# Xharlie/BtcDet

Measured on AMD Instinct MI355X. Metric: scenes/s fwd+bwd KITTI-Car bs=2/GPU (BtcDet hot path), higher is better.
Workload: dtype f32

## Files before the change

btcdet_amd/_lib.py:

```python
import ctypes
import os

import numpy as np
import torch

_HERE = os.path.dirname(os.path.abspath(__file__))
LIB_PATH = os.path.join(_HERE, "libbtcdet_hip.so")
_lib = None

c_i32p = ctypes.POINTER(ctypes.c_int32)
c_f32p = ctypes.POINTER(ctypes.c_float)
vp = ctypes.c_void_p
ci = ctypes.c_int
sz = ctypes.c_size_t

MODE_SUBM, MODE_CONV, MODE_TRANSPOSE = 0, 1, 2


class BtcHipError(RuntimeError):
    pass


class BtcOccConfig(ctypes.Structure):
    _fields_ = [("batch", ctypes.c_int32), ("grid", ctypes.c_int32 * 3), ("sphere_grid", ctypes.c_int32 * 3),
# ... 109 lines not shown
                              sz, vp]),
    "btc_occ_loss_bwd": (ci, [vp, vp, vp, vp, vp, vp, vp, vp, ci, ctypes.c_longlong, ctypes.c_float, vp, vp, vp, vp, vp]),
    "btc_occ_loss_fwd_total": (ci, [vp, vp, vp, vp, vp, vp, vp, vp, ci, ctypes.c_longlong, ctypes.c_float, ctypes.c_float, ctypes.c_float, vp, vp,
                                    vp, sz, vp]),
    "btc_occ_loss_bwd_total": (ci, [vp, vp, vp, vp, vp, vp, vp, vp, ci, ctypes.c_longlong, ctypes.c_float, vp, vp, vp, vp, vp]),
    "btc_dense_split_fwd": (ci, [vp, vp, ci, ci, ci, vp, vp, vp, vp]),
    "btc_occ_prob": (ci, [vp, vp, ci, ctypes.c_longlong, vp, vp]),
    "btc_dense_split_bwd": (ci, [vp, vp, vp, ci, ci, ci, vp, vp, vp]),
    "btc_cat_pad_fwd": (ci, [vp, ci, vp, ci, ctypes.c_longlong, ci, ci, vp, vp]),
    "btc_cat_pad_bwd": (ci, [vp, ci, ctypes.c_longlong, ci, vp, ci, vp, ci, vp]),
    "btc_sumsq2_ws_bytes": (sz, []),
    "btc_sumsq2_fwd": (ci, [vp, ctypes.c_longlong, ci, ctypes.c_double, vp, ctypes.c_longlong, ci, ctypes.c_double, vp, vp, sz, vp]),
    "btc_sumsq2_bwd": (ci, [vp, ctypes.c_longlong, ci, ctypes.c_float, vp, vp, ctypes.c_longlong, ci, ctypes.c_float, vp, vp, vp]),
    "btc_bn_ws_bytes": (sz, [ci]),
    "btc_bn_relu_fwd": (ci, [vp, ci, ci, vp, vp, vp, vp, vp, ctypes.c_float, ctypes.c_float, ci, ci, vp, vp, vp, vp, sz, vp]),
    "btc_spin": (ci, [ci, vp]),
    "btc_bn_relu_bwd": (ci, [vp, vp, vp, ci, ci, vp, vp, vp, ci, ci, vp, vp, vp, vp, sz, vp]),
    "btc_bn_relu_fwd_bf16": (ci, [vp, ci, ci, vp, vp, vp, vp, vp, ctypes.c_float, ctypes.c_float, ci, ci, vp, vp, vp, vp, sz, vp]),
    "btc_bn_relu_bwd_bf16": (ci, [vp, vp, vp, ci, ci, vp, vp, vp, ci, ci, vp, vp, vp, vp, sz, vp]),
    "btc_ball_query": (ci, [vp, vp, vp, vp, ci, ci, ctypes.c_float, ctypes.c_float, ci, vp, vp]),
    "btc_group_points": (ci, [vp, vp, vp, vp, ci, ci, ci, ci, vp, vp]),
    "btc_group_points_grad": (ci, [vp, vp, vp, vp, ci, ci, ci, ci, ci, vp, vp]),
    "btc_furthest_point_sampling": (ci, [vp, ci, ci, ci, vp, vp, vp]),
    "btc_three_nn": (ci, [vp, vp, vp, vp, ci, ci, vp, vp, vp]),
    "btc_three_interpolate": (ci, [vp, vp, vp, ci, ci, vp, vp]),
    "btc_three_interpolate_grad": (ci, [vp, vp, vp, ci, ci, ci, vp, vp]),
    "btc_bn_fuse_ws_bytes": (sz, []),
    "btc_conv_bn_relu_fwd": (ci, [ci, vp, vp, vp, vp, vp, ci, ci, ci, ci, vp, vp, vp, vp, vp, vp, ctypes.c_float, ctypes.c_float, ci, vp, vp, vp, vp, sz, vp, vp]),
    "btc_conv_bn_relu_fwd_src": (ci, [ci, vp, ctypes.c_longlong, vp, vp, vp, vp, ci, ci, ci, ci, vp, vp, vp, vp, vp, vp, ctypes.c_float, ctypes.c_float, ci, vp, vp, vp, vp, sz, vp, vp]),
    "btc_col_sum": (ci, [vp, ci, ci, vp, vp, sz, vp]),
    "btc_col_sum_bf16": (ci, [vp, ci, ci, vp, vp, sz, vp]),
    "btc_occ_targets_ws_bytes": (sz, [ctypes.POINTER(BtcOccConfig)]),
    "btc_occ_backproject_lut": (ci, [ctypes.POINTER(BtcOccConfig), vp, vp]),
    "btc_occ_targets": (ci, [ctypes.POINTER(BtcOccConfig), vp, vp, vp, ci, ci, ci, vp, vp, vp, vp, ci, vp, vp,
                             ctypes.POINTER(BtcOccBuffers), vp, sz, vp]),
}

EXPORTED_SYMBOLS = tuple(_SIGS.keys())

_INFER_SIGS = {
    "btc_conv_bn_eval_fwd": (ci, [ci, vp, ctypes.c_longlong, vp, vp, vp, vp, ci, ci, ci, ci, vp, vp, vp, vp, ctypes.c_float, ci, vp, vp]),
    "btc_det_select_nms_ws_bytes": (sz, [ci, ci]),
    "btc_det_select_nms": (ci, [vp, vp, ci, ci, ci, ci, ci, ctypes.c_float, ctypes.c_float, ci, ci, ci, vp, vp, vp, vp, sz, vp]),
    "btc_det_finish": (ci, [vp, vp, ci, ci, ci, ci, ci, ci, vp, vp, vp, vp, ci, vp, ci, ci, vp, ci, ci, c_f32p, ci, vp, vp, vp, vp, vp, vp]),
    "btc_occ_metrics_ws_bytes": (sz, [ci, ci]),
    "btc_occ_metrics": (ci, [vp, vp, vp, vp, ctypes.c_longlong, vp, vp, vp, ctypes.c_longlong, vp, vp, ci, ci, ci, vp, vp, sz, vp]),
    "btc_kitti_overlaps": (ci, [vp, vp, vp, vp, vp, c_i32p, ci, vp, vp, vp]),
    "btc_kitti_match_tp": (ci, [vp, vp, vp, vp, vp, vp, vp, c_i32p, ci, ci, ci, ci, ci, ci, vp, vp, vp]),
    "btc_kitti_match_stats_ws_bytes": (sz, [ci, ci, ci, ci, ci]),
    "btc_kitti_match_stats": (ci, [vp, vp, vp, vp, vp, vp, vp, vp, vp, vp, vp, c_i32p, ci, ci, ci, ci, ci, ci, ci, vp, vp, vp, sz, vp]),
}

INFER_EXPORTED_SYMBOLS = tuple(_INFER_SIGS.keys())

_AUGMENT_SIGS = {
    "btc_augment_ws_bytes": (sz, [ci, ci, ci]),
    "btc_augment_batch": (ci, [vp, ci, ci, vp, ci, vp, vp, vp, ctypes.c_longlong, vp, vp, vp, vp, ci, ctypes.c_longlong, vp, vp,
                               ctypes.c_longlong, vp, vp, vp, vp, sz, vp]),
    "btc_world_transform": (ci, [vp, ci, ci, vp, ci, vp, vp, vp, vp]),
}

AUGMENT_EXPORTED_SYMBOLS = tuple(_AUGMENT_SIGS.keys())

_BESTMATCH_SIGS = {
    "btc_place_templates": (ci, [vp, ctypes.c_longlong, vp, vp, vp, vp, vp, ci, ci, vp, vp, ctypes.c_longlong, ci, vp, vp]),
}

BESTMATCH_EXPORTED_SYMBOLS = tuple(_BESTMATCH_SIGS.keys())

_FRAMES_SIGS = {
    "btc_fov_crop_ws_bytes": (sz, [ci, ci]),
    "btc_fov_crop": (ci, [vp, ci, ci, vp, ci, vp, ci, vp, vp, vp, vp, sz, vp]),
}

FRAMES_EXPORTED_SYMBOLS = tuple(_FRAMES_SIGS.keys())

_GTDB_SIGS = {
    "btc_cut_objects_ws_bytes": (sz, [ci, ci, ci, ci]),
    "btc_cut_objects": (ci, [vp, ci, ci, vp, ci, vp, vp, vp, ci, ci, ci, vp, vp, vp, vp, sz, vp]),
}

GTDB_EXPORTED_SYMBOLS = tuple(_GTDB_SIGS.keys())


def lib():
    global _lib
    if _lib is None:
        if not os.path.exists(LIB_PATH):
            raise BtcHipError(
                f"{LIB_PATH} not found: build it with `python -c 'import __graft_entry__ as g; g.build()'` "
                f"or `make -C btcdet_amd/csrc` (there is no CPU fallback for the hot path)")
        L = ctypes.CDLL(LIB_PATH)
        for name, (res, args) in (list(_SIGS.items()) + list(_INFER_SIGS.items()) + list(_AUGMENT_SIGS.items()) + list(_BESTMATCH_SIGS.items()) +
                                  list(_FRAMES_SIGS.items()) + list(_GTDB_SIGS.items())):
            fn = getattr(L, name)
            fn.restype = res
            fn.argtypes = args
        for kv in filter(None, os.environ.get("BTC_TUNE", "").split(",")):
            k, v = kv.split("=")
            if L.btc_tune_set(int(k), int(v)) != 0:
                raise BtcHipError("BTC_TUNE: bad entry %r" % kv)
        _lib = L
    return _lib


_fast = False


def fast():
    global _fast
    if _fast is False:
        _fast = None
        if os.environ.get("BTC_FASTPATH", "1") != "0":
            try:
                lib()
                from . import _btcfast
                if _btcfast.abi_version() == lib().btc_version():
                    _fast = _btcfast
            except ImportError:
                _fast = None
    return _fast


def check(rc, what):
    if rc != 0:
        msg = lib().btc_last_error().decode("utf-8", "replace")
        raise BtcHipError(f"{what} failed (code {rc}): {msg}")


_raw_stream = torch._C._cuda_getCurrentRawStream
_cur_device = torch._C._cuda_getDevice


def stream_ptr():
    return _raw_stream(_cur_device())


def ptr(t):
    if t is None:
        return None
    if not (t.is_cuda and t.is_contiguous()):
        raise BtcHipError("expected a contiguous tensor on the GPU (HIP) device")
    return t.data_ptr()


_I3_CACHE = {}


def i3(v):
    if isinstance(v, (int, np.integer)):
        key = (int(v),) * 3
    else:
        key = tuple(int(x) for x in np.asarray(v).reshape(-1))
        if len(key) != 3:
            raise BtcHipError(f"expected 3 values, got {v!r}")
    a = _I3_CACHE.get(key)
    if a is None:
        a = np.ascontiguousarray(np.array(key, dtype=np.int32))
        a.setflags(write=False)
        a_ptr = a.ctypes.data_as(c_i32p)
        _I3_CACHE[key] = a
        _I3P_CACHE[id(a)] = (a, a_ptr)
    return a


_I3P_CACHE = {}


def i3p(a):
    hit = _I3P_CACHE.get(id(a))
    if hit is not None and hit[0] is a:
        return hit[1]
    return a.ctypes.data_as(c_i32p)


def f32p(a):
    return a.ctypes.data_as(c_f32p)
# ... 5 lines not shown
```

btcdet_amd/backbones_3d.py:

```python
import os
from functools import partial

import torch
import torch.nn as nn

from . import spconv


def post_act_block(in_channels, out_channels, kernel_size, indice_key=None, stride=1, padding=0, conv_type='subm',
                   norm_fn=None, defaultvalue=1.0, activation=nn.ReLU):
    if conv_type == 'subm':
        conv = spconv.SubMConv3d(in_channels, out_channels, kernel_size, bias=False, indice_key=indice_key)
    elif conv_type == 'subm2d':
        conv = spconv.SubMConv2d(in_channels, out_channels, kernel_size, bias=False, indice_key=indice_key)
    elif conv_type == 'spconv':
        conv = spconv.SparseConv3d(in_channels, out_channels, kernel_size, stride=stride, padding=padding, bias=False,
                                   indice_key=indice_key)
    elif conv_type == 'fixspconv':
        conv = fixSparseConv3d(in_channels, out_channels, kernel_size, stride=stride, padding=padding, bias=False,
                               indice_key=indice_key, defaultvalue=defaultvalue)
        conv.requires_grad_(False)
    elif conv_type == 'spdeconv':
        conv = spconv.SparseConvTranspose3d(in_channels, out_channels, kernel_size, stride=stride, padding=padding,
                                            bias=False, indice_key=indice_key)
# ... 226 lines not shown

    def _stage(self, stage, x, ready):
        sl = ready[0].stage_slices.get(id(stage)) if ready is not None else None
        if sl is not None:
            chain = stage._chain_plan(x, ready[1][sl[0]:sl[1]])
            if chain is not None:
                return stage._run_chain(x, *chain)
        return stage(x)

    def _stages(self, stages, x, ready):
        for stage in stages:
            x = self._stage(stage, x, ready)
        return x

    def _build_occ_net(self, kind, i):
        n = self.occ_code_num
        key = 'spconv%d' % (i + 1)
        pad = 1 if i < 3 else (1, 1, 1)
        kw = {'maxpool': dict(k=3, conv_type='maxpool'), 'weight': dict(k=3, conv_type='spconv'),
              'fix': dict(k=3, conv_type='fixspconv', defaultvalue=1.0 / 27),
              'avgpool': dict(k=2, conv_type='fixspconv', defaultvalue=1)}[kind]
        k = kw.pop('k')
        setattr(self, 'occ_conv%d' % (i + 1), spconv.SparseSequential(
            post_act_block(n, n, k, norm_fn=None, stride=2, padding=pad, indice_key=key, **kw)))

    def _build_combine_net(self, norm_fn, c, comb_type):
        sp = dict(stride=2, conv_type='spconv')
        self.down2 = _seq([(c[1], c[1], 3, dict(padding=1, indice_key='spconv3', **sp)),
                           (c[1], c[2], 3, dict(padding=(0, 1, 1), indice_key='spconv4', **sp))], norm_fn)
        self.down3 = _seq([(c[2], c[2], 3, dict(padding=(0, 1, 1), indice_key='spconv4', **sp))], norm_fn)
        cat = c[2] * 2 + c[3]
        if comb_type == "big_combine":
            self.down_combine = _seq([(cat, c[3] * 2, 3, dict(padding=1, indice_key='subm4')),
                                      (c[3] * 2, c[3] * 2, 3, dict(padding=1, indice_key='subm4'))], norm_fn)
        elif comb_type == "combine":
            self.down_combine = _seq([(cat, c[3] * 2, 3, dict(padding=1, indice_key='subm4')),
                                      (c[3] * 2, c[3] * 2, 3, dict(stride=[1, 2, 2], padding=(1, 1, 1), indice_key='spconv5',
                                                                   conv_type='spconv')),
                                      (c[3] * 2, c[3] * 2, 3, dict(padding=1, indice_key='subm5'))], norm_fn)
        elif comb_type == "big_bev_combine":
            self.squeezeBev = _seq([(c[4], c[3], (2, 1, 1), dict(stride=(2, 1, 1), padding=0, indice_key='subm_down2',
                                                                  conv_type='spconv'))], norm_fn)
            self.down_combine = _seq([(cat + c[3], c[3] * 2, 3, dict(padding=1, indice_key='subm4')),
                                      (c[3] * 2, c[3] * 2, 3, dict(padding=1, indice_key='subm4'))], norm_fn)

    @staticmethod
    def sparse_cat(input_lst, pad=False):
        xrep, xocc = input_lst
        if pad:
            from .spconv import ops as sp_ops
            xrep.features = sp_ops.cat_features(xrep.features, xocc.features)
        else:
            xrep.features = torch.cat((xrep.features, xocc.features.to(xrep.features.dtype)), dim=1)
        return xrep

    @staticmethod
    def apply_att(x, att_conv):
        a = att_conv(x)
        x.features = x.features * a.features + x.features
        return x

    def suqeeze(self, feat, i, kind):
        if kind == "None":
            return None
        if kind == "3D":
            return feat
        conv = getattr(self, "squeeze_z_conv{}".format(i), None)
        dense = feat.dense()
        B, C, Z, Y, X = list(dense.shape)
        inds = torch.unique(torch.cat([feat.indices[..., 0:1], feat.indices[..., 2:]], dim=-1), dim=0).long()
        pix = dense.reshape(B, C * Z, Y, X)[inds[..., 0], :, inds[..., 1], inds[..., 2]]
        return conv(spconv.SparseConvTensor(features=pix, indices=inds.int(), spatial_shape=[Y, X], batch_size=B)).dense()

    @staticmethod
    def compress_height(t):
        d = t.dense()
        N, C, D, H, W = d.shape
        return d.view(N, C * D, H, W)

    def res_combine(self, x2, x3, x4, bev, out_feat_type="combine", ready=None):
        if getattr(self, "down3", None) is None:
            return None
        x2, x3 = self._stage(self.down2, x2, ready), self._stage(self.down3, x3, ready)
        if out_feat_type == "big_bev_combine":
            bev2d = self.compress_height(self._stage(self.squeezeBev, bev, ready))
            x4.features = torch.cat((x2.features, x3.features, x4.features,
                                     _BevGather.apply(bev2d, x4.indices, tuple(x4.spatial_shape), x4.batch_size).to(x4.features.dtype)), dim=1)
        else:
            x4.features = torch.cat((x2.features, x3.features, x4.features), dim=1)
        return self._stage(self.down_combine, x4, ready)

    @staticmethod
    def _coords_i32(batch_dict):
        from .vfe import i32_twin
        coords = batch_dict['voxel_coords']
        tw = i32_twin(batch_dict, coords)
        return tw if tw is not None else coords.int()

    def prefetch_geometry(self, batch_dict):
        coords = self._coords_i32(batch_dict)
        if not coords.is_cuda or coords.shape[0] == 0:
            return batch_dict
        indice_dict = {}
        walk = self._walk_geometry(coords, batch_dict['batch_size'], indice_dict, allow_async=False)
        if isinstance(walk, tuple) and walk[0] == "done":
            batch_dict['det_geometry'] = (coords, indice_dict, walk)
        return batch_dict

    def forward(self, batch_dict):
        coords = self._coords_i32(batch_dict)
        feats = batch_dict['voxel_features']
        if self.feature_dtype is not None and feats.shape[1] % 16 == 0:
            feats = feats.to(self.feature_dtype)
        bs = batch_dict['batch_size']
        x = spconv.SparseConvTensor(features=feats, indices=coords, spatial_shape=self.sparse_shape, batch_size=bs)
        pre = batch_dict.pop('det_geometry', None)
        if pre is not None and pre[0] is coords:
            x.indice_dict = pre[1]
            walk = pre[2]
        else:
            walk = self._walk_geometry(coords, bs, x.indice_dict)
        n_occ = len(self.occ_conv_exec)
        ready = None
        if FAST_STAGES and isinstance(walk, tuple) and walk[0] == "done":
            ready = self._finish_walk(walk, x.indice_dict)
        merge_first = ready is not None and not (n_occ > 0 and self.occ_conv_exec[0])
        x1 = _to_feature_dtype(self._stage(self.conv1, x, ready), self.feature_dtype)
        if merge_first:
            x1 = self._stage(self.conv1_combine, x1, ready)
        occ = None
        if n_occ > 0:
            occ = spconv.SparseConvTensor(features=batch_dict["occ_voxel_features"], indices=coords,
                                          spatial_shape=self.sparse_shape, batch_size=bs)
            occ.indice_dict["__geometry_cache__"] = x.indice_dict.setdefault("__geometry_cache__", {})
            if self.occ_conv_exec[0]:
                x1 = self.sparse_cat([x1, occ], pad=not self.out_att[0])
                if self.out_att[0]:
                    x1 = self.apply_att(x1, self.att_conv1)
        if not merge_first:
            x1 = self._stage(self.conv1_combine, x1, ready)
        if ready is None:
            ready = self._finish_walk(walk, x.indice_dict)
            if not FAST_STAGES:
                ready = None
        levels = [x1]
        cur = x1
        for lvl in (1, 2, 3):
            if not (n_occ > lvl):
                cur = self._stages([getattr(self, 'conv%d' % (lvl + 1)), getattr(self, 'conv%d_combine' % (lvl + 1))], cur, ready)
                levels.append(cur)
                continue
            cur = self._stage(getattr(self, 'conv%d' % (lvl + 1)), cur, ready)
            if n_occ > lvl:
                occ = getattr(self, 'occ_conv%d' % (lvl + 1))(occ)
                if self.occ_conv_exec[lvl]:
                    cur = self.sparse_cat([cur, occ], pad=not self.out_att[lvl])
                    if self.out_att[lvl]:
                        cur = self.apply_att(cur, getattr(self, 'att_conv%d' % (lvl + 1)))
            cur = self._stage(getattr(self, 'conv%d_combine' % (lvl + 1)), cur, ready)
            levels.append(cur)
        x1, x2, x3, x4 = levels
        out = self._stage(self.conv_out, x4, ready)
        batch_dict.update({'encoded_spconv_tensor': out, 'encoded_spconv_tensor_stride': 8})
        batch_dict['__level_rows__'] = {'det_L0': int(x1.features.shape[0]), 'det_L1': int(x2.features.shape[0]),
                                        'det_L2': int(x3.features.shape[0]), 'det_L3': int(x4.features.shape[0]),
                                        'det_out': int(out.features.shape[0])}
        batch_dict.update({'multi_scale_3d_features': {
            'x_conv1': self.suqeeze(x1, 1, self.out_feat_type[0]),
            'x_conv2': self.suqeeze(x2, 2, self.out_feat_type[1]),
            'x_conv3': self.suqeeze(x3, 3, self.out_feat_type[2]),
            'x_conv4': self.suqeeze(x4, 4, self.out_feat_type[3]),
            'x_combine': self.res_combine(x2, x3, x4, out, out_feat_type=self.out_feat_type[4], ready=ready),
# ... 163 lines not shown
```

btcdet_amd/spconv/ops.py:

```python
import os

import numpy as np
import torch

from .. import _lib
from .._lib import MODE_CONV, MODE_SUBM, MODE_TRANSPOSE, check, fast, i3, i3p, lib, ptr, stream_ptr, workspace


class LaunchProfile(object):

    def __init__(self):
        self.records = []

    def span(self, name, nbytes, flops, info=None):
        return _Span(self, name, nbytes, flops, info)

    def details(self):
        return [(r[0], r[1].elapsed_time(r[2]), r[3], r[4], r[5] if len(r) > 5 else None) for r in self.records]

    def summary(self):
        out = {}
        for name, e0, e1, nbytes, flops in [r[:5] for r in self.records]:
            d = out.setdefault(name, {"launches": 0, "ms": 0.0, "bytes": 0, "flops": 0})
            d["launches"] += 1
            d["ms"] += e0.elapsed_time(e1)
            d["bytes"] += nbytes
            d["flops"] += flops
        return out


class _Span(object):
    def __init__(self, prof, name, nbytes, flops, info=None):
        self.prof, self.name, self.nbytes, self.flops, self.info = prof, name, nbytes, flops, info

    def __enter__(self):
        self.e0 = torch.cuda.Event(enable_timing=True)
        self.e1 = torch.cuda.Event(enable_timing=True)
        self.e0.record()

    def __exit__(self, *a):
        self.e1.record()
        self.prof.records.append((self.name, self.e0, self.e1, self.nbytes, self.flops, self.info))


class _NoSpan(object):
    def __enter__(self):
        return None

    def __exit__(self, *a):
        return False


PROFILE = None
CAPTURE = None
OVERLAP_WGRAD = True
_STREAMS = {}


def _wgrad_stream(device):
    key = device.index if device.index is not None else torch.cuda.current_device()
    st = _STREAMS.get(key)
    if st is None:
        st = _STREAMS[key] = torch.cuda.Stream(device=device)
    return st


_NOSPAN = _NoSpan()


def _span(name, cost_fn, args):
    if PROFILE is None:
        return _NOSPAN
    r = cost_fn(*args)
    return PROFILE.span(name, r[0], r[1], r[2] if len(r) > 2 else None)


def _num_pairs(nbr):
    n = getattr(nbr, "_btc_pairs", None)
    if n is None:
        n = int((nbr >= 0).sum().item())
        nbr._btc_pairs = n
    return n
# ... 502 lines not shown
        sh = i3([int(v) for v in spatial_shape])
        dense = torch.zeros((int(batch_size), C, int(sh[0]), int(sh[1]), int(sh[2])), dtype=torch.float32,
                            device=features.device)
        check(lib().btc_dense_fwd(ptr(features), ptr(indices), n, C, i3p(sh), ptr(dense), stream_ptr()), "btc_dense_fwd")
        ctx.save_for_backward(indices)
        ctx.sh = sh
        ctx.nc = (n, C)
        return dense

    @staticmethod
    def backward(ctx, grad_dense):
        (indices,) = ctx.saved_tensors
        n, C = ctx.nc
        grad_dense = _f32c(grad_dense)
        dfeat = torch.empty((n, C), dtype=torch.float32, device=grad_dense.device)
        check(lib().btc_dense_bwd(ptr(grad_dense), ptr(indices), n, C, i3p(ctx.sh), ptr(dfeat), stream_ptr()),
              "btc_dense_bwd")
        return dfeat, None, None, None


class DenseSplitFunction(torch.autograd.Function):

    @staticmethod
    def forward(ctx, features, indices, batch_size, spatial_shape, ca):
        features = _f32c(features)
        indices = _as_idx(indices)
        n, C = features.shape
        cb = C - int(ca)
        sh = i3([int(v) for v in spatial_shape])
        B, vol = int(batch_size), int(sh[0]) * int(sh[1]) * int(sh[2])
        flat = torch.zeros((B * C * vol,), dtype=torch.float32, device=features.device)
        da = flat[:B * ca * vol].view(B, ca, int(sh[0]), int(sh[1]), int(sh[2]))
        db = flat[B * ca * vol:].view(B, cb, int(sh[0]), int(sh[1]), int(sh[2]))
        check(lib().btc_dense_split_fwd(ptr(features), ptr(indices), n, int(ca), cb, i3p(sh), ptr(da), ptr(db), stream_ptr()), "btc_dense_split_fwd")
        ctx.save_for_backward(indices)
        ctx.meta = (sh, n, int(ca), cb)
        return da, db

    @staticmethod
    def backward(ctx, ga, gb):
        (indices,) = ctx.saved_tensors
        sh, n, ca, cb = ctx.meta
        ga = _f32c(ga) if ga is not None else None
        gb = _f32c(gb) if gb is not None else None
        dev = (ga if ga is not None else gb).device
        dfeat = torch.empty((n, ca + cb), dtype=torch.float32, device=dev)
        check(lib().btc_dense_split_bwd(ptr(ga), ptr(gb), ptr(indices), n, ca, cb, i3p(sh), ptr(dfeat), stream_ptr()), "btc_dense_split_bwd")
        return dfeat, None, None, None, None


def dense_split(features, indices, batch_size, spatial_shape, ca):
    return DenseSplitFunction.apply(features, indices, batch_size, spatial_shape, ca)


class CatPadFunction(torch.autograd.Function):

    @staticmethod
    def forward(ctx, a, b, cout):
        a, b = a.contiguous(), b.contiguous()
        n, ca, cb = a.shape[0], a.shape[1], b.shape[1]
        out = torch.empty((n, int(cout)), dtype=a.dtype, device=a.device)
        check(lib().btc_cat_pad_fwd(ptr(a), ca, ptr(b), cb, n, int(cout), a.element_size(), ptr(out), stream_ptr()), "btc_cat_pad_fwd")
        ctx.meta = (n, ca, cb, int(cout), a.dtype)
        return out

    @staticmethod
    def backward(ctx, g):
        n, ca, cb, cout, dt = ctx.meta
        g = (g if g.dtype == dt else g.to(dt)).contiguous()
        da = torch.empty((n, ca), dtype=dt, device=g.device)
        db = torch.empty((n, cb), dtype=dt, device=g.device)
        check(lib().btc_cat_pad_bwd(ptr(g), cout, n, g.element_size(), ptr(da), ca, ptr(db), cb, stream_ptr()), "btc_cat_pad_bwd")
        return da, db, None


def cat_features(a, b):
    b = b.to(a.dtype)
    cc = a.shape[1] + b.shape[1]
    if a.is_cuda and a.dtype in (torch.float32, torch.bfloat16) and a.dim() == 2 and a.shape[0] > 0 and pads_in_channels(cc):
        return CatPadFunction.apply(a, b, cc + _pad_amount(cc, a.dtype))
    return torch.cat((a, b), dim=1)


PAD_CHANNELS = 0


def pads_in_channels(cin):
    return cin > 16 and cin % 16 != 0


def _pad_amount(cin, dtype):
    return (-cin) % (PAD_CHANNELS or (32 if dtype == torch.float32 else 16))


def _pad_in_channels(features, weight):
    cin = weight.shape[-2]
    if features.is_cuda and pads_in_channels(cin):
        pad = _pad_amount(cin, features.dtype)
        if features.shape[1] == cin + pad:
            return features, torch.nn.functional.pad(weight, (0, 0, 0, pad))
        return torch.nn.functional.pad(features, (0, pad)), torch.nn.functional.pad(weight, (0, 0, 0, pad))
    return features, weight


def indice_conv(features, weight, bias, rulebook, inverse=False, keep_fp32=False):
    features, weight = _pad_in_channels(features, weight)
    if features.dtype == torch.bfloat16 and (weight.shape[-2] % 16 or weight.shape[-1] % 16):
        out = indice_conv(features.float(), weight, bias, rulebook, inverse)
        return out if keep_fp32 else out.to(torch.bfloat16)
    if inverse:
        return SparseConvFunction.apply(features, weight, bias, rulebook.nbr_in, rulebook.nbr_out, rulebook.order_in, rulebook.order_out)
    return SparseConvFunction.apply(features, weight, bias, rulebook.nbr_out, rulebook.map_bwd, rulebook.order_out, rulebook.order_in)


def indice_conv_bn_relu(features, weight, bias, rulebook, bn, relu, inverse=False):
    features, weight = _pad_in_channels(features, weight)
    if features.dtype == torch.bfloat16 and (weight.shape[-2] % 16 or weight.shape[-1] % 16):
        from . import fused_bn
        return fused_bn.batch_norm_relu(bn, indice_conv(features, weight, bias, rulebook, inverse), relu)
    training = bn.training or not bn.track_running_stats
    nbt = bn.num_batches_tracked if (bn.training and bn.track_running_stats) else None
    rm = bn.running_mean if bn.track_running_stats else None
    rv = bn.running_var if bn.track_running_stats else None
    maps = (rulebook.nbr_in, rulebook.nbr_out) if inverse else (rulebook.nbr_out, rulebook.map_bwd)
    ords = (rulebook.order_in, rulebook.order_out) if inverse else (rulebook.order_out, rulebook.order_in)
    if PROFILE is None and CAPTURE is None and features.is_cuda and maps[0].shape[0] >= 1:
        from . import fused_bn
        if fused_bn.eval_fold_wanted(features, weight, bias, bn):
            with torch.no_grad():
                return fused_bn.conv_bn_eval_forward(_actc(features), _f32c(weight), _f32c(bias) if bias is not None else None, maps[0], ords[0],
                                                     bn.weight, bn.bias, rm, rv, bn.eps, relu)
    F = fast() if (PROFILE is None and CAPTURE is None and NATIVE_AUTOGRAD) else None
    if F is not None and features.is_cuda:
        from . import fused_bn
        ws, need = fused_bn._ws(features.device, weight.shape[-1])
        return F.conv_bn_relu(_actc(features), _f32c(weight), bias, maps[0], maps[1], ords[0], ords[1], bn.weight, bn.bias, rm, rv, nbt, bool(training or rm is None),
                              float(bn.momentum), float(bn.eps), bool(relu), ws, need, bool(_overlap_ok(maps[0].shape[0])), bool(weight.is_leaf))
    return SparseConvBNReLUFunction.apply(features, weight, bias, maps[0], maps[1], bn.weight, bn.bias, rm, rv, nbt, training, bn.momentum,
                                          bn.eps, relu, ords[0], ords[1])


def indice_maxpool(features, rulebook):
    if features.dtype == torch.bfloat16:
        return indice_maxpool(features.float(), rulebook).to(torch.bfloat16)
    return SparseMaxPoolFunction.apply(features, rulebook.nbr_out, rulebook.nbr_in)
```

Measured before the change: 588.7.

## Fuse feature concat and sparse BEV gather into one combine-rows kernel

Replaces the torch.cat of the down2/down3/x4 features, plus the densify-and-gather of the squeezed BEV tensor, with one HIP kernel. For each output row it copies the source segments and looks up matching BEV cells with a wave-cooperative search over the sorted sparse BEV indices. The backward pass scatters gradients back to the sources and accumulates BEV gradients by searching the other way. This removes the dense BEV materialization and several launches and copies. The costs are per-row search work and reliance on the index lists being sorted.

```diff
diff --git a/btcdet_amd/_lib.py b/btcdet_amd/_lib.py
--- a/btcdet_amd/_lib.py
+++ b/btcdet_amd/_lib.py
@@ -215,6 +215,13 @@
 
 GTDB_EXPORTED_SYMBOLS = tuple(_GTDB_SIGS.keys())
 
+_COMBINE_SIGS = {
+    "btc_combine_rows_fwd": (ci, [vp, vp, ci, ci, vp, vp, vp, ci, ci, ci, ci, vp, vp]),
+    "btc_combine_rows_bwd": (ci, [vp, vp, ci, ci, vp, ci, vp, ci, ci, ci, ci, vp, vp, vp]),
+}
+
+COMBINE_EXPORTED_SYMBOLS = tuple(_COMBINE_SIGS.keys())
+
 
 def lib():
     global _lib
@@ -225,7 +232,7 @@
                 f"or `make -C btcdet_amd/csrc` (there is no CPU fallback for the hot path)")
         L = ctypes.CDLL(LIB_PATH)
         for name, (res, args) in (list(_SIGS.items()) + list(_INFER_SIGS.items()) + list(_AUGMENT_SIGS.items()) + list(_BESTMATCH_SIGS.items()) +
-                                  list(_FRAMES_SIGS.items()) + list(_GTDB_SIGS.items())):
+                                  list(_FRAMES_SIGS.items()) + list(_GTDB_SIGS.items()) + list(_COMBINE_SIGS.items())):
             fn = getattr(L, name)
             fn.restype = res
             fn.argtypes = args
diff --git a/btcdet_amd/backbones_3d.py b/btcdet_amd/backbones_3d.py
--- a/btcdet_amd/backbones_3d.py
+++ b/btcdet_amd/backbones_3d.py
@@ -332,12 +332,9 @@
         if getattr(self, "down3", None) is None:
             return None
         x2, x3 = self._stage(self.down2, x2, ready), self._stage(self.down3, x3, ready)
-        if out_feat_type == "big_bev_combine":
-            bev2d = self.compress_height(self._stage(self.squeezeBev, bev, ready))
-            x4.features = torch.cat((x2.features, x3.features, x4.features,
-                                     _BevGather.apply(bev2d, x4.indices, tuple(x4.spatial_shape), x4.batch_size).to(x4.features.dtype)), dim=1)
-        else:
-            x4.features = torch.cat((x2.features, x3.features, x4.features), dim=1)
+        from .spconv import ops as sp_ops
+        squeezed = self._stage(self.squeezeBev, bev, ready) if out_feat_type == "big_bev_combine" else None
+        x4.features = sp_ops.combine_rows((x2.features, x3.features, x4.features), x4.indices, x4.spatial_shape, x4.batch_size, squeezed)
         return self._stage(self.down_combine, x4, ready)
 
     @staticmethod
diff --git a/btcdet_amd/csrc/combine.hip b/btcdet_amd/csrc/combine.hip
--- /dev/null
+++ b/btcdet_amd/csrc/combine.hip
@@ -0,0 +1,217 @@
+#include "btc_common.h"
+#include "../../include/btcdet_hip_combine.h"
+
+namespace {
+
+struct CombineSegs {
+  void* p[BTC_COMBINE_MAX_SRC];
+  int w[BTC_COMBINE_MAX_SRC];
+  int n;
+  int W;
+};
+
+__device__ __forceinline__ int find_cells(const int4* __restrict__ idx, int n, int b, int nkeys, int y, int x, int lane) {
+  int G = 64;
+  while (G * nkeys > 64) G >>= 1;
+  const int grp = lane / G, sub = lane - grp * G;
+  const int z = grp;
+  const unsigned long long gmask = G == 64 ? ~0ull : ((1ull << G) - 1);
+  int lo = 0, hi = grp < nkeys ? n : 0;
+  while (__any(lo < hi)) {
+    const bool open = lo < hi;
+    const long long len = hi - lo;
+    bool less = false;
+    if (open) {
+      const int4 q = idx[lo + (int)(((long long)(sub + 1) * len) / (G + 1))];
+      less = q.x != b ? q.x < b : (q.y != z ? q.y < z : (q.z != y ? q.z < y : q.w < x));
+    }
+    const int k = __popcll((__ballot(less) >> (grp * G)) & gmask);
+    if (open) {
+      const int lo0 = lo;
+      if (k > 0) lo = lo0 + (int)(((long long)k * len) / (G + 1)) + 1;
+      if (k < G) hi = lo0 + (int)(((long long)(k + 1) * len) / (G + 1));
+    }
+  }
+  int row = -1;
+  if (grp < nkeys && lo < n) {
+    const int4 q = idx[lo];
+    if (q.x == b && q.y == z && q.z == y && q.w == x) row = lo;
+  }
+  const int got = __shfl(row, (lane < nkeys ? lane : 0) * G, 64);
+  return lane < nkeys ? got : -1;
+}
+
+template <typename U, bool TO_WIDE>
+__device__ __forceinline__ void move_segments(const CombineSegs& s, int per_u, size_t r, U* __restrict__ wide_row, int lane) {
+  int off = 0;
+#pragma unroll
+  for (int i = 0; i < BTC_COMBINE_MAX_SRC; ++i) {
+    if (i < s.n) {
+      const int w = s.w[i] / per_u;
+      U* seg = (U*)s.p[i] + r * (size_t)w;
+      for (int j = lane; j < w; j += 64) {
+        if (TO_WIDE) wide_row[off + j] = seg[j];
+        else seg[j] = wide_row[off + j];
+      }
+      off += w;
+    }
+  }
+}
+
+template <typename T, bool VEC>
+__global__ __launch_bounds__(256) void combine_rows_fwd_k(CombineSegs s, int M, const int4* __restrict__ idx, const T* __restrict__ bev,
+                                                          const int4* __restrict__ bev_idx, int Mb, int C, int Db, T* __restrict__ out) {
+  const int lane = threadIdx.x & 63;
+  const long long r = (long long)blockIdx.x * 4 + (threadIdx.x >> 6);
+  if (r >= M) return;
+  const size_t pitch = (size_t)s.W + (size_t)C * Db;
+  T* orow = out + (size_t)r * pitch;
+  if (VEC) move_segments<uint4, true>(s, 16 / (int)sizeof(T), (size_t)r, (uint4*)orow, lane);
+  else move_segments<T, true>(s, 1, (size_t)r, orow, lane);
+  if (C == 0) return;
+  const int4 q = idx[r];
+  const int mine = find_cells(bev_idx, Mb, q.x, Db, q.z, q.w, lane);
+  if (VEC) {
+    const int src = __shfl(mine, 0, 64);
+    const int nv = C / (16 / (int)sizeof(T));
+    uint4* g = (uint4*)(orow + s.W);
+    const uint4* b = (const uint4*)(bev + (size_t)(src < 0 ? 0 : src) * C);
+    for (int j = lane; j < nv; j += 64) g[j] = src < 0 ? make_uint4(0, 0, 0, 0) : b[j];
+  } else {
+    T* g = orow + s.W;
+    const int total = C * Db;
+    for (int j0 = 0; j0 < total; j0 += 64) {
+      const int j = j0 + lane;
+      const int c = j / Db, d = j - c * Db;
+      const int src = __shfl(mine, d, 64);
+      if (j < total) g[j] = src < 0 ? (T)0 : bev[(size_t)src * C + c];
+    }
+  }
+}
+
+template <typename T, bool VEC>
+__global__ __launch_bounds__(256) void combine_rows_bwd_k(CombineSegs s, int M, const int4* __restrict__ idx, int Dz, const T* __restrict__ dout,
+                                                          const int4* __restrict__ bev_idx, int Mb, int C, int Db, T* __restrict__ dbev) {
+  const int lane = threadIdx.x & 63;
+  const long long wv = (long long)blockIdx.x * 4 + (threadIdx.x >> 6);
+  const size_t pitch = (size_t)s.W + (size_t)C * Db;
+  if (wv < M) {
+    T* grow = const_cast<T*>(dout) + (size_t)wv * pitch;
+    if (VEC) move_segments<uint4, false>(s, 16 / (int)sizeof(T), (size_t)wv, (uint4*)grow, lane);
+    else move_segments<T, false>(s, 1, (size_t)wv, grow, lane);
+    return;
+  }
+  const long long rb = wv - M;
+  if (C == 0 || rb >= Mb) return;
+  const int4 q = bev_idx[rb];
+  const bool d_ok = q.y >= 0 && q.y < Db;
+  const int mine = d_ok ? find_cells(idx, M, q.x, Dz, q.z, q.w, lane) : -1;
+  const unsigned long long have = __ballot(mine >= 0);
+  const T* g = dout + s.W + (d_ok ? q.y : 0);
+  for (int c0 = 0; c0 < C; c0 += 64) {
+    const int c = c0 + lane;
+    float acc = 0.f;
+    for (unsigned long long m = have; m; m &= m - 1) {
+      const int z = __builtin_ctzll(m);
+      const int r = __shfl(mine, z, 64);
+      if (c < C) {
+        const T v = g[(size_t)r * pitch + (size_t)c * Db];
+        if (sizeof(T) == 2) acc += btc_bf16_to_f32((unsigned short)v);
+        else acc += __uint_as_float((unsigned)v);
+      }
+    }
+    if (c < C) {
+      if (sizeof(T) == 2) dbev[(size_t)rb * C + c] = (T)btc_f32_to_bf16(acc);
+      else dbev[(size_t)rb * C + c] = (T)__float_as_uint(acc);
+    }
+  }
+}
+
+bool aligned16(const void* p) { return (reinterpret_cast<uintptr_t>(p) & 15) == 0; }
+
+int combine_args(const char* who, void* const* h_ptr, const int32_t* h_width, int n_src, int M, const int32_t* idx, const void* bev,
+                 const int32_t* bev_idx, int Mb, int C, int Db, int elem_bytes, const void* wide, CombineSegs* s, bool* vec) {
+  BTC_CHECK_ARG(elem_bytes == 4 || elem_bytes == 2, "%s: elem_bytes must be 2 or 4", who);
+  BTC_CHECK_ARG(n_src >= 0 && n_src <= BTC_COMBINE_MAX_SRC, "%s: n_src must be 0 .. %d", who, BTC_COMBINE_MAX_SRC);
+  BTC_CHECK_ARG(n_src == 0 || (h_ptr && h_width), "%s: NULL h_src / h_width", who);
+  BTC_CHECK_ARG(M >= 0 && C >= 0, "%s: bad sizes", who);
+  if (C > 0) {
+    BTC_CHECK_ARG(Mb >= 0, "%s: Mb < 0", who);
+    BTC_CHECK_ARG(Db >= 1 && Db <= 64, "%s: Db must be 1 .. 64", who);
+    BTC_CHECK_ARG(Mb == 0 || (bev && bev_idx), "%s: NULL bev operand with Mb > 0", who);
+    BTC_CHECK_ARG(M == 0 || idx, "%s: NULL idx", who);
+    BTC_CHECK_ARG(aligned16(idx) && aligned16(bev_idx), "%s: the index lists must be 16-byte aligned", who);
+  }
+  *vec = (C == 0 || Db == 1) && (C * elem_bytes) % 16 == 0 && aligned16(bev) && aligned16(wide);
+  s->n = n_src;
+  s->W = 0;
+  for (int i = 0; i < BTC_COMBINE_MAX_SRC; ++i) {
+    s->p[i] = nullptr;
+    s->w[i] = 0;
+  }
+  for (int i = 0; i < n_src; ++i) {
+    BTC_CHECK_ARG(h_width[i] >= 1, "%s: width %d < 1", who, i);
+    BTC_CHECK_ARG(M == 0 || h_ptr[i], "%s: NULL matrix %d", who, i);
+    s->p[i] = h_ptr[i];
+    s->w[i] = h_width[i];
+    s->W += h_width[i];
+    *vec = *vec && (h_width[i] * elem_bytes) % 16 == 0 && aligned16(h_ptr[i]);
+  }
+  BTC_CHECK_ARG(s->W + (long long)C * (C > 0 ? Db : 0) > 0, "%s: an output row has no columns", who);
+  BTC_CHECK_ARG(M == 0 || wide, "%s: NULL out / dout", who);
+  return BTC_OK;
+}
+
+}
+
+extern "C" int btc_combine_rows_fwd(const void* const* h_src, const int32_t* h_width, int n_src, int M, const int32_t* idx, const void* bev,
+                                    const int32_t* bev_idx, int Mb, int C, int Db, int elem_bytes, void* out, void* stream_) {
+  hipStream_t stream = (hipStream_t)stream_;
+  CombineSegs s;
+  bool vec;
+  const int rc = combine_args("btc_combine_rows_fwd", (void* const*)h_src, h_width, n_src, M, idx, bev, bev_idx, Mb, C, Db, elem_bytes, out, &s, &vec);
+  if (rc != BTC_OK) return rc;
+  if (M == 0) return BTC_OK;
+  if (C == 0) Mb = 0, Db = 1;
+  const int grid = btc_cdiv(M, 4);
+  const int4 *ix = (const int4*)idx, *bx = (const int4*)bev_idx;
+  if (elem_bytes == 4) {
+    if (vec) combine_rows_fwd_k<unsigned, true><<<grid, 256, 0, stream>>>(s, M, ix, (const unsigned*)bev, bx, Mb, C, Db, (unsigned*)out);
+    else combine_rows_fwd_k<unsigned, false><<<grid, 256, 0, stream>>>(s, M, ix, (const unsigned*)bev, bx, Mb, C, Db, (unsigned*)out);
+  } else {
+    if (vec)
+      combine_rows_fwd_k<unsigned short, true><<<grid, 256, 0, stream>>>(s, M, ix, (const unsigned short*)bev, bx, Mb, C, Db, (unsigned short*)out);
+    else
+      combine_rows_fwd_k<unsigned short, false><<<grid, 256, 0, stream>>>(s, M, ix, (const unsigned short*)bev, bx, Mb, C, Db, (unsigned short*)out);
+  }
+  BTC_LAUNCH_CHECK();
+  return BTC_OK;
+}
+
+extern "C" int btc_combine_rows_bwd(const void* dout, const int32_t* h_width, int n_src, int M, const int32_t* idx, int Dz, const int32_t* bev_idx,
+                                    int Mb, int C, int Db, int elem_bytes, void* const* h_dsrc, void* dbev, void* stream_) {
+  hipStream_t stream = (hipStream_t)stream_;
+  CombineSegs s;
+  bool vec;
+  const int rc = combine_args("btc_combine_rows_bwd", h_dsrc, h_width, n_src, M, idx, dbev, bev_idx, Mb, C, Db, elem_bytes, dout, &s, &vec);
+  if (rc != BTC_OK) return rc;
+  BTC_CHECK_ARG(C == 0 || (Dz >= 1 && Dz <= 64), "btc_combine_rows_bwd: Dz must be 1 .. 64");
+  if (C == 0) Mb = 0, Db = 1;
+  const long long waves = (long long)M + Mb;
+  if (waves == 0) return BTC_OK;
+  const int grid = btc_cdiv(waves, 4);
+  const int4 *ix = (const int4*)idx, *bx = (const int4*)bev_idx;
+  if (elem_bytes == 4) {
+    if (vec) combine_rows_bwd_k<unsigned, true><<<grid, 256, 0, stream>>>(s, M, ix, Dz, (const unsigned*)dout, bx, Mb, C, Db, (unsigned*)dbev);
+    else combine_rows_bwd_k<unsigned, false><<<grid, 256, 0, stream>>>(s, M, ix, Dz, (const unsigned*)dout, bx, Mb, C, Db, (unsigned*)dbev);
+  } else {
+    if (vec)
+      combine_rows_bwd_k<unsigned short, true><<<grid, 256, 0, stream>>>(s, M, ix, Dz, (const unsigned short*)dout, bx, Mb, C, Db,
+                                                                         (unsigned short*)dbev);
+    else
+      combine_rows_bwd_k<unsigned short, false><<<grid, 256, 0, stream>>>(s, M, ix, Dz, (const unsigned short*)dout, bx, Mb, C, Db,
+                                                                          (unsigned short*)dbev);
+  }
+  BTC_LAUNCH_CHECK();
+  return BTC_OK;
+}
diff --git a/btcdet_amd/spconv/ops.py b/btcdet_amd/spconv/ops.py
--- a/btcdet_amd/spconv/ops.py
+++ b/btcdet_amd/spconv/ops.py
@@ -1,3 +1,4 @@
+import ctypes
 import os
 
 import numpy as np
@@ -666,6 +667,71 @@
     return torch.cat((a, b), dim=1)
 
 
+class CombineRowsFunction(torch.autograd.Function):
+
+    @staticmethod
+    def forward(ctx, indices, bev_indices, dz, db, bev, *srcs):
+        srcs = [s.contiguous() for s in srcs]
+        like = bev if bev is not None else srcs[0]
+        M, n = int(indices.shape[0]), len(srcs)
+        widths = [int(s.shape[1]) for s in srcs]
+        C, Mb = (int(bev.shape[1]), int(bev.shape[0])) if bev is not None else (0, 0)
+        if bev is not None:
+            bev = bev.contiguous()
+        h_width = (ctypes.c_int32 * max(n, 1))(*widths)
+        out = torch.empty((M, sum(widths) + C * int(db)), dtype=like.dtype, device=like.device)
+        check(lib().btc_combine_rows_fwd((ctypes.c_void_p * max(n, 1))(*[ptr(s) for s in srcs]), h_width, n, M, ptr(indices), ptr(bev),
+                                         ptr(bev_indices) if C else None, Mb, C, int(db), like.element_size(), ptr(out), stream_ptr()),
+              "btc_combine_rows_fwd")
+        ctx.save_for_backward(indices, bev_indices if C else None)
+        ctx.meta = (widths, h_width, M, Mb, C, int(dz), int(db), like.dtype)
+        return out
+
+    @staticmethod
+    def backward(ctx, g):
+        indices, bev_indices = ctx.saved_tensors
+        widths, h_width, M, Mb, C, dz, db, dt = ctx.meta
+        g = (g if g.dtype == dt else g.to(dt)).contiguous()
+        dsrc = [torch.empty((M, w), dtype=dt, device=g.device) for w in widths]
+        dbev = torch.empty((Mb, C), dtype=dt, device=g.device) if C else None
+        n = len(widths)
+        check(lib().btc_combine_rows_bwd(ptr(g), h_width, n, M, ptr(indices), dz, ptr(bev_indices), Mb, C, db, g.element_size(),
+                                         (ctypes.c_void_p * max(n, 1))(*[ptr(d) for d in dsrc]), ptr(dbev), stream_ptr()),
+              "btc_combine_rows_bwd")
+        return (None, None, None, None, dbev) + tuple(dsrc)
+
+
+COMBINE_MAX_SRC = 4
+COMBINE_NATIVE = True
+
+
+def combine_rows(srcs, indices, spatial_shape, batch_size, bev=None):
+    srcs = list(srcs)
+    feats = srcs + ([bev.features] if bev is not None else [])
+    dt = feats[0].dtype if feats else None
+    native = (COMBINE_NATIVE and 0 < len(feats) and len(srcs) <= COMBINE_MAX_SRC and dt in (torch.float32, torch.bfloat16)
+              and all(f.is_cuda and f.dim() == 2 and f.dtype == dt for f in feats) and indices.is_cuda and indices.dim() == 2
+              and (bev is None or (bev.indices.shape[1] == 4 and 1 <= int(bev.spatial_shape[0]) <= 64 and 1 <= int(spatial_shape[0]) <= 64)))
+    if native:
+        return CombineRowsFunction.apply(_as_idx(indices), _as_idx(bev.indices) if bev is not None else None, int(spatial_shape[0]),
+                                         int(bev.spatial_shape[0]) if bev is not None else 1, bev.features if bev is not None else None, *srcs)
+    if bev is None:
+        return torch.cat(srcs, dim=1)
+    out_dt = srcs[-1].dtype if srcs else dt
+    if bev.features.is_cuda:
+        from ..backbones_3d import _BevGather
+        d = bev.dense()
+        N, C, D, H, W = d.shape
+        g = _BevGather.apply(d.view(N, C * D, H, W), indices, tuple(spatial_shape), batch_size)
+    else:
+        C, (D, H, W) = bev.features.shape[1], [int(v) for v in bev.spatial_shape]
+        bi, ii = bev.indices.long(), indices.long()
+        d = bev.features.new_zeros((int(batch_size), C, D, H, W))
+        d[bi[:, 0], :, bi[:, 1], bi[:, 2], bi[:, 3]] = bev.features
+        g = d.view(int(batch_size), C * D, H, W)[ii[:, 0], :, ii[:, 2], ii[:, 3]]
+    return torch.cat(srcs + [g.to(out_dt)], dim=1)
+
+
 PAD_CHANNELS = 0
 
 
diff --git a/include/btcdet_hip_combine.h b/include/btcdet_hip_combine.h
--- /dev/null
+++ b/include/btcdet_hip_combine.h
@@ -0,0 +1,23 @@
+#ifndef BTCDET_HIP_COMBINE_H
+#define BTCDET_HIP_COMBINE_H
+
+#include <stddef.h>
+#include <stdint.h>
+
+#include "btcdet_hip.h"
+
+#define BTC_COMBINE_MAX_SRC 4
+
+#ifdef __cplusplus
+extern "C" {
+#endif
+
+int btc_combine_rows_fwd(const void* const* h_src, const int32_t* h_width, int n_src, int M, const int32_t* idx,
+                         const void* bev, const int32_t* bev_idx, int Mb, int C, int Db, int elem_bytes, void* out, void* stream);
+int btc_combine_rows_bwd(const void* dout, const int32_t* h_width, int n_src, int M, const int32_t* idx, int Dz,
+                         const int32_t* bev_idx, int Mb, int C, int Db, int elem_bytes, void* const* h_dsrc, void* dbev, void* stream);
+
+#ifdef __cplusplus
+}
+#endif
+#endif
```

Measured after the change: 603.1, median of 6. 1.02x the previous value.
